# ViTAE-Transformer/SAMRS

Measured on AMD Instinct MI355X. Metric: images/sec (1024^2, vit_h, 32 boxes/img) SAM box->mask, higher is better.
Workload: dtype f16

## Files before the change

samrs_amd/csrc/common.h:

```cpp
#pragma once
#include <hip/hip_runtime.h>
#include <stdint.h>

typedef __attribute__((ext_vector_type(8))) __bf16 bf16x8_t;
typedef __attribute__((ext_vector_type(8))) _Float16 f16x8_t;
typedef __attribute__((ext_vector_type(4))) float f32x4_t;
typedef __attribute__((ext_vector_type(16))) float f32x16_t;

#define SAMRS_WAVE 64

enum { PREC_BF16 = 0, PREC_F16 = 1 };

template <int PREC>
struct ET;

template <>
struct ET<PREC_BF16> {
    static __device__ __forceinline__ uint16_t from_float(float f) {
        __bf16 b = (__bf16)f;
        return __builtin_bit_cast(uint16_t, b);
    }
    static __device__ __forceinline__ float to_float(uint16_t u) {
        return __builtin_bit_cast(float, (uint32_t)u << 16);
    }
// ... 39 lines not shown
}
template <int PREC>
__device__ __forceinline__ uint32_t pack2(float lo, float hi) {
    if (PREC == PREC_F16) {
        lo = __builtin_amdgcn_fmed3f(lo, -65504.0f, 65504.0f);
        hi = __builtin_amdgcn_fmed3f(hi, -65504.0f, 65504.0f);
    }
    return pack2_fast<PREC>(lo, hi);
}

template <int PREC>
__device__ __forceinline__ void split2_pack(float a, float b, uint32_t& hi, uint32_t& lo) {
    hi = pack2<PREC>(a, b);
    const float ha = ET<PREC>::to_float((uint16_t)(hi & 0xffffu)), hb = ET<PREC>::to_float((uint16_t)(hi >> 16));
    lo = pack2<PREC>(a - ha, b - hb);
}

constexpr int MXK = 256;
constexpr int MX_SA_BYTES = 2048, MX_SB_BYTES = 4096;

__device__ __forceinline__ uint32_t fp4_code(float v) {
    const float a = fabsf(v);
    const float step = a >= 4.f ? 2.f : a >= 2.f ? 1.f : 0.5f;
    const float q = fminf(rintf(a / step) * step, 6.f);
    const int idx = (int)(q * 2.f);
    const uint32_t code = idx <= 4 ? (uint32_t)idx : (uint32_t)(idx >> 2) + 4u;
    return code | (v < 0.f ? 8u : 0u);
}
__device__ __forceinline__ int mx_scale_byte(float amax) {
    const int e = (int)((__float_as_uint(amax) >> 23) & 0xffu);
// ... 126 lines not shown
```

samrs_amd/csrc/decoder_kernels.hip:

```cpp
#include "common.h"
#include "kernels.h"
#include "postprocess_value.h"

namespace {

constexpr float TWO_PI = 6.283185307179586f;

__device__ __forceinline__ float pe_channel(const float* __restrict__ gauss, float cx01, float cy01, int ch, int half) {
    const int f = ch < half ? ch : ch - half;
    const float vx = 2.0f * cx01 - 1.0f, vy = 2.0f * cy01 - 1.0f;
    const float a = TWO_PI * (vx * gauss[f] + vy * gauss[half + f]);
    return ch < half ? sinf(a) : cosf(a);
}

__global__ void prompt_tokens_kernel(PromptParams p, float* __restrict__ tokens, float* __restrict__ tokens2, int T, int C) {
    const int j = blockIdx.x, b = blockIdx.y, ch = threadIdx.x;
    const int half = C / 2;
    const bool has_pts = p.point_coords != nullptr;
    const bool has_box = p.boxes != nullptr;
    const int npt = has_pts ? p.n_points + (has_box ? 0 : 1) : 0;
    float v;
    if (j == 0) {
        v = p.iou_token[ch];
    } else if (j < 5) {
// ... 373 lines not shown
        m = mn;
    }
    const float inv = 1.0f / l;
    uint4 o0, o1;
    o0.x = pack2<PREC>(acc[0] * inv, acc[1] * inv);   o0.y = pack2<PREC>(acc[2] * inv, acc[3] * inv);
    o0.z = pack2<PREC>(acc[4] * inv, acc[5] * inv);   o0.w = pack2<PREC>(acc[6] * inv, acc[7] * inv);
    o1.x = pack2<PREC>(acc[8] * inv, acc[9] * inv);   o1.y = pack2<PREC>(acc[10] * inv, acc[11] * inv);
    o1.z = pack2<PREC>(acc[12] * inv, acc[13] * inv); o1.w = pack2<PREC>(acc[14] * inv, acc[15] * inv);
    uint16_t* orow = out + ((size_t)b * tokens + tok) * Ci + h * HD;
    *reinterpret_cast<uint4*>(orow) = o0;
    *reinterpret_cast<uint4*>(orow + 8) = o1;
}

constexpr int I2TF_ROWS = 32;
constexpr int I2TF_AST = 136;

template <int PREC, bool SPLIT>
__global__ __launch_bounds__(256, 2) void i2t_fused_kernel(const uint16_t* __restrict__ qi, int ld, long q_bstride,
                                                        const int* __restrict__ slot_of, const float* __restrict__ kt, const float* __restrict__ vt,
                                                        const uint16_t* __restrict__ w, const uint16_t* __restrict__ w_lo,
                                                        const float* __restrict__ bias,
                                                        const float* __restrict__ resid, long r_bstride,
                                                        const float* __restrict__ gamma, const float* __restrict__ beta, float eps,
                                                        float* __restrict__ outF, uint16_t* __restrict__ outE,
                                                        uint16_t* __restrict__ outE_lo, int T, int tokens, int groups_per_block) {
    constexpr int HD = 16, HEADS = 8, CI = 128, CO = 256, NWV = 4;
    constexpr int KRS = HEADS * I2T_HS;
    extern __shared__ __attribute__((aligned(16))) unsigned char smraw[];
    float* sk = reinterpret_cast<float*>(smraw);
    float* sv = sk + T * KRS;
    float* sp = sv + T * KRS;
    float* ex = sp + 3 * CO;
    uint16_t* At = reinterpret_cast<uint16_t*>(ex + 2 * NWV * I2TF_ROWS);
    uint16_t* Al = At + I2TF_ROWS * I2TF_AST;
    const int tid = threadIdx.x, lane = tid & 63, wave = tid >> 6;
    const int fr = lane & 15, fq = lane >> 4;
    const int b = blockIdx.y;
    for (int i = tid; i < T * CI; i += 256) {
        const int j = i / CI, c = i % CI;
        sk[j * KRS + (c / HD) * I2T_HS + c % HD] = kt[(size_t)b * T * CI + i];
        sv[j * KRS + (c / HD) * I2T_HS + c % HD] = vt[(size_t)b * T * CI + i];
    }
    for (int i = tid; i < CO; i += 256) { sp[i] = bias[i]; sp[CO + i] = gamma[i]; sp[2 * CO + i] = beta[i]; }
    uint4 wf[4][4], wl[SPLIT ? 4 : 1][4];
#pragma unroll
    for (int i = 0; i < 4; ++i)
#pragma unroll
        for (int ks = 0; ks < 4; ++ks) {
            const size_t o = (size_t)(wave * 64 + i * 16 + fr) * CI + ks * 32 + fq * 8;
            wf[i][ks] = *reinterpret_cast<const uint4*>(w + o);
            if constexpr (SPLIT) wl[i][ks] = *reinterpret_cast<const uint4*>(w_lo + o);
        }
    __syncthreads();

    const int tr = tid >> 3, h = tid & 7;
    const int g0 = blockIdx.x * groups_per_block;
    const int ib = slot_of ? slot_of[b] : b;
    const uint16_t* qbase = qi + (size_t)ib * q_bstride * ld + (size_t)tr * ld + h * HD;
    uint4 q0 = make_uint4(0u, 0u, 0u, 0u), q1 = q0;
    if (g0 * I2TF_ROWS < tokens) {
        q0 = *reinterpret_cast<const uint4*>(qbase + (size_t)g0 * I2TF_ROWS * ld);
        q1 = *reinterpret_cast<const uint4*>(qbase + (size_t)g0 * I2TF_ROWS * ld + 8);
    }
    for (int g = g0; g < g0 + groups_per_block; ++g) {
        const int row0 = g * I2TF_ROWS;
        if (row0 >= tokens) break;
        float4 rs[2][4];
#pragma unroll
        for (int mt = 0; mt < 2; ++mt)
#pragma unroll
            for (int i = 0; i < 4; ++i)
                rs[mt][i] = *reinterpret_cast<const float4*>(resid + ((size_t)ib * r_bstride + row0 + mt * 16 + fr) * CO + wave * 64 + i * 16 + 4 * fq);
        {
            const uint32_t qw[8] = {q0.x, q0.y, q0.z, q0.w, q1.x, q1.y, q1.z, q1.w};
            float qf[HD];
#pragma unroll
            for (int c = 0; c < 8; ++c) {
                qf[2 * c] = ET<PREC>::to_float((uint16_t)(qw[c] & 0xffffu)) * 0.25f;
                qf[2 * c + 1] = ET<PREC>::to_float((uint16_t)(qw[c] >> 16)) * 0.25f;
            }
            float m = -INFINITY, l = 0.f, acc[HD];
#pragma unroll
            for (int c = 0; c < HD; ++c) acc[c] = 0.f;
            for (int j = 0; j < T; ++j) {
                float kr[HD], vr[HD];
#pragma unroll
                for (int c4 = 0; c4 < HD / 4; ++c4) {
// ... 11 lines not shown
#pragma unroll
                for (int c = 0; c < HD; ++c) acc[c] = acc[c] * corr + pj * vr[c];
                m = mn;
            }
            const float inv = 1.0f / l;
            uint32_t oh[8], ol[8];
#pragma unroll
            for (int c = 0; c < 8; ++c) split2_pack<PREC>(acc[2 * c] * inv, acc[2 * c + 1] * inv, oh[c], ol[c]);
            *reinterpret_cast<uint4*>(At + tr * I2TF_AST + h * HD) = make_uint4(oh[0], oh[1], oh[2], oh[3]);
            *reinterpret_cast<uint4*>(At + tr * I2TF_AST + h * HD + 8) = make_uint4(oh[4], oh[5], oh[6], oh[7]);
            if constexpr (SPLIT) {
                *reinterpret_cast<uint4*>(Al + tr * I2TF_AST + h * HD) = make_uint4(ol[0], ol[1], ol[2], ol[3]);
                *reinterpret_cast<uint4*>(Al + tr * I2TF_AST + h * HD + 8) = make_uint4(ol[4], ol[5], ol[6], ol[7]);
            }
        }
        __syncthreads();
        if (g + 1 < g0 + groups_per_block && (g + 1) * I2TF_ROWS < tokens) {
            q0 = *reinterpret_cast<const uint4*>(qbase + (size_t)(g + 1) * I2TF_ROWS * ld);
            q1 = *reinterpret_cast<const uint4*>(qbase + (size_t)(g + 1) * I2TF_ROWS * ld + 8);
        }
        float v[2][4][4];
        float s1[2];
#pragma unroll
        for (int mt = 0; mt < 2; ++mt) {
            uint4 af[4], al[SPLIT ? 4 : 1];
#pragma unroll
            for (int ks = 0; ks < 4; ++ks) {
                af[ks] = *reinterpret_cast<const uint4*>(At + (mt * 16 + fr) * I2TF_AST + ks * 32 + fq * 8);
                if constexpr (SPLIT) al[ks] = *reinterpret_cast<const uint4*>(Al + (mt * 16 + fr) * I2TF_AST + ks * 32 + fq * 8);
            }
            s1[mt] = 0.f;
#pragma unroll
            for (int i = 0; i < 4; ++i) {
                f32x4_t a = {0.f, 0.f, 0.f, 0.f};
                if constexpr (SPLIT) {
                    f32x4_t c = {0.f, 0.f, 0.f, 0.f};
#pragma unroll
                    for (int ks = 0; ks < 4; ++ks) c = ET<PREC>::mfma16(wf[i][ks], al[ks], c);
#pragma unroll
                    for (int ks = 0; ks < 4; ++ks) c = ET<PREC>::mfma16(wl[i][ks], af[ks], c);
                    a = c;
                }
#pragma unroll
                for (int ks = 0; ks < 4; ++ks) a = ET<PREC>::mfma16(wf[i][ks], af[ks], a);
                const float4 bb = *reinterpret_cast<const float4*>(sp + wave * 64 + i * 16 + 4 * fq);
                v[mt][i][0] = (a[0] + bb.x) + rs[mt][i].x; v[mt][i][1] = (a[1] + bb.y) + rs[mt][i].y;
                v[mt][i][2] = (a[2] + bb.z) + rs[mt][i].z; v[mt][i][3] = (a[3] + bb.w) + rs[mt][i].w;
                s1[mt] += (v[mt][i][0] + v[mt][i][1]) + (v[mt][i][2] + v[mt][i][3]);
            }
        }
#pragma unroll
        for (int mt = 0; mt < 2; ++mt) {
            s1[mt] += __shfl_xor(s1[mt], 16, 64);
            s1[mt] += __shfl_xor(s1[mt], 32, 64);
            if (fq == 0) ex[wave * I2TF_ROWS + mt * 16 + fr] = s1[mt];
        }
        __syncthreads();
        float mean[2], s2[2];
#pragma unroll
        for (int mt = 0; mt < 2; ++mt) {
            const int r = mt * 16 + fr;
            mean[mt] = ((ex[r] + ex[I2TF_ROWS + r]) + (ex[2 * I2TF_ROWS + r] + ex[3 * I2TF_ROWS + r])) * (1.0f / CO);
            s2[mt] = 0.f;
#pragma unroll
            for (int i = 0; i < 4; ++i)
#pragma unroll
                for (int r4 = 0; r4 < 4; ++r4) { v[mt][i][r4] -= mean[mt]; s2[mt] += v[mt][i][r4] * v[mt][i][r4]; }
            s2[mt] += __shfl_xor(s2[mt], 16, 64);
            s2[mt] += __shfl_xor(s2[mt], 32, 64);
            if (fq == 0) ex[NWV * I2TF_ROWS + wave * I2TF_ROWS + r] = s2[mt];
        }
        __syncthreads();
#pragma unroll
        for (int mt = 0; mt < 2; ++mt) {
            const int r = mt * 16 + fr;
            const float* e2 = ex + NWV * I2TF_ROWS;
            const float rstd = 1.0f / sqrtf(((e2[r] + e2[I2TF_ROWS + r]) + (e2[2 * I2TF_ROWS + r] + e2[3 * I2TF_ROWS + r])) * (1.0f / CO) + eps);
            const size_t orow = (size_t)b * tokens + row0 + r;
#pragma unroll
            for (int i = 0; i < 4; ++i) {
                const int n = wave * 64 + i * 16 + 4 * fq;
                const float4 gm = *reinterpret_cast<const float4*>(sp + CO + n), bt = *reinterpret_cast<const float4*>(sp + 2 * CO + n);
                const float y0 = v[mt][i][0] * rstd * gm.x + bt.x, y1 = v[mt][i][1] * rstd * gm.y + bt.y;
                const float y2 = v[mt][i][2] * rstd * gm.z + bt.z, y3 = v[mt][i][3] * rstd * gm.w + bt.w;
                if (outF) *reinterpret_cast<float4*>(outF + orow * CO + n) = make_float4(y0, y1, y2, y3);
                uint2 o, lo;
                split2_pack<PREC>(y0, y1, o.x, lo.x);
                split2_pack<PREC>(y2, y3, o.y, lo.y);
                *reinterpret_cast<uint2*>(outE + orow * CO + n) = o;
                if (outE_lo) *reinterpret_cast<uint2*>(outE_lo + orow * CO + n) = lo;
            }
        }
    }
}

template <int PREC>
__global__ __launch_bounds__(256) void group_ln_gelu_kernel(const float* __restrict__ in, const float* __restrict__ gamma,
                                                            const float* __restrict__ beta, float eps,
                                                            uint16_t* __restrict__ out, long rows) {
    const int lane = threadIdx.x & 63;
    const long row = (long)blockIdx.x * 4 + (threadIdx.x >> 6);
    if (row >= rows) return;
    const float4 v = reinterpret_cast<const float4*>(in + row * 256)[lane];
    float s = (v.x + v.y) + (v.z + v.w);
#pragma unroll
    for (int off = 8; off > 0; off >>= 1) s += __shfl_xor(s, off, 64);
    const float mean = s * (1.0f / 64.0f);
    const float a = v.x - mean, b = v.y - mean, c = v.z - mean, d = v.w - mean;
// ... 581 lines not shown
        i2t_attention_kernel<PREC_BF16><<<g, b, sh, s>>>((const uint16_t*)qi, ld, bstride, kt, vt, (uint16_t*)out, T, tokens, Ci);
    else
        i2t_attention_kernel<PREC_F16><<<g, b, sh, s>>>((const uint16_t*)qi, ld, bstride, kt, vt, (uint16_t*)out, T, tokens, Ci);
    return hipGetLastError();
}
hipError_t launch_i2t_fused(int prec, const void* qi, int ld, long q_bstride, const float* kt, const float* vt, const void* w,
                            const void* w_lo, const float* bias, const float* resid, long r_bstride, const float* gamma,
                            const float* beta, float eps, float* outF, void* outE, void* outE_lo, int n, int T, int tokens, int Ci,
                            int C, hipStream_t s, const int* slot_of) {
    if (Ci != 128 || C != 256 || T < 1 || T > TOK_MAX || tokens % I2TF_ROWS) return hipErrorInvalidValue;
    const int groups = tokens / I2TF_ROWS;
    int gpb = 4;
    while (gpb > 1 && groups % gpb) gpb >>= 1;
    dim3 g(groups / gpb, n), b(256);
    const bool split = w_lo != nullptr;
    const size_t sh = (size_t)(2 * T * 8 * I2T_HS + 3 * 256 + 2 * 4 * I2TF_ROWS) * sizeof(float) +
                      (size_t)(split ? 2 : 1) * I2TF_ROWS * I2TF_AST * 2;
#define I2TF_LAUNCH(P, S)                                                                                                       \
    i2t_fused_kernel<P, S><<<g, b, sh, s>>>((const uint16_t*)qi, ld, q_bstride, slot_of, kt, vt, (const uint16_t*)w, (const uint16_t*)w_lo, \
                                           bias, resid, r_bstride, gamma, beta, eps, outF, (uint16_t*)outE, (uint16_t*)outE_lo, T, \
                                           tokens, gpb)
    if (prec == PREC_BF16) { if (split) I2TF_LAUNCH(PREC_BF16, true); else I2TF_LAUNCH(PREC_BF16, false); }
    else { if (split) I2TF_LAUNCH(PREC_F16, true); else I2TF_LAUNCH(PREC_F16, false); }
#undef I2TF_LAUNCH
    return hipGetLastError();
}
hipError_t launch_group_ln_gelu(int prec, const float* in, const float* gamma, const float* beta, float eps,
                                void* out, long rows, int groups, int gsize, hipStream_t s) {
    if (groups != 4 || gsize != 64) return hipErrorInvalidValue;
    const int blocks = (int)((rows + 3) / 4);
    if (prec == PREC_BF16) group_ln_gelu_kernel<PREC_BF16><<<blocks, 256, 0, s>>>(in, gamma, beta, eps, (uint16_t*)out, rows);
    else group_ln_gelu_kernel<PREC_F16><<<blocks, 256, 0, s>>>(in, gamma, beta, eps, (uint16_t*)out, rows);
    return hipGetLastError();
}
hipError_t launch_mask_product(int prec, const void* up2, const float* hyper, float* low, int n, int grid,
                               int n_mask_tokens, int sel0, int n_sel, hipStream_t s) {
    if (n_sel > 4 || n_sel < 1) return hipErrorInvalidValue;
    const int S = 4 * grid;
// ... 79 lines not shown
```

samrs_amd/csrc/encoder_kernels.hip:

```cpp
#include "common.h"
#include "kernels.h"

namespace {

__constant__ float c_mean[3] = {123.675f, 116.28f, 103.53f};
__constant__ float c_std[3] = {58.395f, 57.12f, 57.375f};

template <int PREC>
__global__ void patch_im2col_kernel(const uint8_t* __restrict__ img, uint16_t* __restrict__ A, uint16_t* __restrict__ A_lo,
                                    int n_images, int in_h, int in_w, int grid, int patch) {
    const int P2 = patch * patch;
    const int halves = patch / 8;
    const long total = (long)n_images * grid * grid * patch * halves;
    const long t = (long)blockIdx.x * blockDim.x + threadIdx.x;
    if (t >= total) return;
    const int half = t % halves;
    long u = t / halves;
    const int ky = u % patch; u /= patch;
    const int px = u % grid; u /= grid;
    const int py = u % grid;
    const int im = u / grid;
    const int y = py * patch + ky, x0 = px * patch + half * 8;
    float v[3][8];
#pragma unroll
// ... 437 lines not shown
        ah = fmaxf(ah, xhalf_partner(ah));
        al = fmaxf(al, xhalf_partner(al));
        const int bh = mx_scale_byte(ah), bl = mx_scale_byte(al);
        const uint2 ch = make_uint2(fp4_pack8(h, bh), fp4_pack8(h + 8, bh)), cl = make_uint2(fp4_pack8(l, bl), fp4_pack8(l + 8, bl));
        *reinterpret_cast<uint2*>(qh + dt * 16 + 8 * hh) = ch;
        *reinterpret_cast<uint2*>(ql + dt * 16 + 8 * hh) = cl;
        if (hh == 0) {
            const size_t si = mx_scale_index(false, (int)row, head * DT + dt, nst4);
            mx.s_hi[si] = (unsigned char)bh;
            mx.s_lo[si] = (unsigned char)bl;
        }
    }
}

template <int HD>
struct WinCfg {
    static constexpr int WS = 14, N = WS * WS, TK = 2 * WS, NT = N / TK, NP = NT * 32;
    static constexpr int DT = (HD + 31) / 32;
    static constexpr bool ONES = SAMRS_WIN_ONES && DT * 32 > HD;
    __device__ static constexpr int lds_key(int key) { return key + (32 - TK) * (key / TK); }
    static constexpr int VSTR = 228;
    static constexpr int NW = 8, THREADS = NW * 64;
    static constexpr int SSTR = 33;
    static constexpr int K_BYTES = NP * HD * 2;
    static constexpr int VT_BYTES = DT * 32 * VSTR * 2;
    static constexpr int S_BYTES = NW * 32 * SSTR * 4;
    static constexpr int TAB_BYTES = 2 * 32 * HD * 2;
    static constexpr int MAX_D = 1280;
    static constexpr int BIAS_BYTES = 2 * MAX_D * 2;
    static constexpr int LDS_BYTES = K_BYTES + VT_BYTES + S_BYTES + TAB_BYTES + BIAS_BYTES;
};

template <int PREC, int HD, int LO = 0 , int PIPE = 0>
__global__ __launch_bounds__(512) void window_attention_kernel(
    const uint16_t* __restrict__ qkv, const float* __restrict__ qkv_bias, const float* __restrict__ rel_h,
    const float* __restrict__ rel_w, uint16_t* __restrict__ out, int grid, int heads, int n_items,
    uint16_t* __restrict__ out_lo = nullptr , MxOut mx = MxOut(),
    uint32_t lo_heads = 0xffffffffu ,
    int dense = 1 ) {
    using C = WinCfg<HD>;
    constexpr int KS = HD / 16;
    constexpr bool PL = (PIPE & 1) != 0;
    extern __shared__ __attribute__((aligned(16))) unsigned char smem[];
    uint16_t* Ks = reinterpret_cast<uint16_t*>(smem);
    uint16_t* Vt = reinterpret_cast<uint16_t*>(smem + C::K_BYTES);
    float* Scr = reinterpret_cast<float*>(smem + C::K_BYTES + C::VT_BYTES);
    uint16_t* Tab = reinterpret_cast<uint16_t*>(smem + C::K_BYTES + C::VT_BYTES + C::S_BYTES);
    uint16_t* Bia = Tab + 2 * 32 * HD;
// ... 113 lines not shown
        } else WIN_LOAD_V((g_) - 1 - NGK < PV ? (g_) - 1 - NGK : 0);                                                 \
    } while (0)
#define WIN_ISSUE(it_)                                                                                               \
    do {                                                                                                             \
        WIN_HEAD(it_);                                                                                               \
        _Pragma("unroll") for (int g_ = 0; g_ < NGRP; ++g_) WIN_GROUP(g_);                                           \
        if constexpr (PL) WIN_LOAD_Q();                                                                              \
    } while (0)

    __syncthreads();
    if constexpr ((PIPE & 2) != 0) {
        if (__builtin_amdgcn_readfirstlane(threadIdx.x) >= 256) __builtin_amdgcn_s_setprio(1);
    }
    int it = blockIdx.x;
#ifdef WIN_TIMING
    unsigned long long wph[6] = {0, 0, 0, 0, 0, 0}, wprev = __builtin_amdgcn_s_memtime();
    const unsigned long long wstart = wprev;
    int n_done = 0;
#define WIN_STAMP(i_) { const unsigned long long tn_ = __builtin_amdgcn_s_memtime(); wph[i_] += tn_ - wprev; wprev = tn_; }
#else
#define WIN_STAMP(i_)
#endif
    if (it < n_items) WIN_ISSUE(it);
    for (; it < n_items; it += gridDim.x) {
        __syncthreads();
        WIN_STAMP(0)
        if (__any(n_pad != 0u)) {
#pragma unroll
            for (int i = 0; i < PK; ++i) {
                const uint4 kb = *reinterpret_cast<const uint4*>(Bia + n_head * HD + ((tid + i * C::THREADS) % CH) * 8);
                kreg[i] = sel4((n_pad >> i) & 1u, kb, kreg[i]);
// ... 31 lines not shown
        const int qc = min(q, n_nq - 1), qh = slot_row(qc, n_vw), qw = qc - qh * n_vw;
        WIN_STAMP(1)
        __syncthreads();
        WIN_STAMP(2)
        const bool has_next = it + (int)gridDim.x < n_items;
        if (has_next) {
            if (wave_u >= n_strips) WIN_ISSUE(it + (int)gridDim.x);
            else WIN_HEAD(it + (int)gridDim.x);
        }
        WIN_STAMP(3)
#ifdef WIN_TIMING
        ++n_done;
#endif
        if (wave_u >= n_strips) continue;

        float* scr = Scr + wave * 32 * C::SSTR + ql * C::SSTR;
        float RH[PL ? 1 : C::WS], BW[16];
        float* rhs = scr;
        {
            const f32x16_t th = tile_times_qT<PREC, HD>(Tab, lane, qf);
            if constexpr (PL) {
                const f32x16_t tw = tile_times_qT<PREC, HD>(Tab + 32 * HD, lane, qf);
#pragma unroll
                for (int r = 0; r < 16; ++r) scr[acc_row(r, hh)] = tw[r];
                wave_lds_sync();
#pragma unroll
                for (int r = 0; r < 16; ++r) {
                    const int c = acc_row(r, hh);
                    BW[r] = c < C::TK ? scr[qw - c % C::WS + C::WS - 1] * LOG2E_F : -INFINITY;
                }
                wave_lds_sync();
// ... 87 lines not shown
            for (int u = 0; u < 2; ++u) {
                const uint4 pb = pack_p<PREC>(S, u);
#pragma unroll
                for (int dt = 0; dt < C::DT; ++dt) {
                    const uint4 va = load_vt_frag(Vt + (dt * 32 + ql) * C::VSTR + 32 * t, u, hh);
                    O[dt] = ET<PREC>::mfma32(va, pb, O[dt]);
                }
            }
        }
        if constexpr (C::ONES) l_run = ones_row_sum<HD, C::DT>(O, hh);
        else l_run += xhalf_partner(l_run);

#ifdef WIN_TIMING
        asm volatile("" :: "v"(O[0][0]), "v"(O[C::DT - 1][15]), "v"(l_run), "v"(qin), "v"(im), "v"(head));
        WIN_STAMP(5)
        continue;
#endif
        if (qin) {
            const float inv = 1.0f / l_run;
            const size_t orow_i = (size_t)im * img_rows + (size_t)(qoff / (3 * D));
            const size_t obase = orow_i * D + head * HD;
            uint16_t* orow = out + obase;
            if constexpr (LO == 2) store_attention_row_mx<PREC, HD, C::DT>(O, inv, orow, hh, mx, orow_i, head, heads);
            else
#pragma unroll
            for (int dt = 0; dt < C::DT; ++dt)
#pragma unroll
                for (int g = 0; g < 4; ++g) {
                    const int d0 = 32 * dt + 8 * g + 4 * hh;
                    if (d0 < HD) {
                        uint2 o;
                        o.x = pack2_fast<PREC>(O[dt][4 * g + 0] * inv, O[dt][4 * g + 1] * inv);
                        o.y = pack2_fast<PREC>(O[dt][4 * g + 2] * inv, O[dt][4 * g + 3] * inv);
                        *reinterpret_cast<uint2*>(orow + d0) = o;
                        if constexpr (LO == 1) {
                            if ((lo_heads >> (head & 31)) & 1u) {
                                uint2 h, l;
                                split2_pack<PREC>(O[dt][4 * g + 0] * inv, O[dt][4 * g + 1] * inv, h.x, l.x);
                                split2_pack<PREC>(O[dt][4 * g + 2] * inv, O[dt][4 * g + 3] * inv, h.y, l.y);
                                *reinterpret_cast<uint2*>(out_lo + obase + d0) = l;
                            }
                        }
                    }
                }
        }
    }
#ifdef WIN_TIMING
    if (lane == 0) {
        unsigned long long* tp = reinterpret_cast<unsigned long long*>(out) + ((size_t)blockIdx.x * 8 + wave) * 8;
        for (int i = 0; i < 6; ++i) tp[i] = wph[i];
        tp[6] = __builtin_amdgcn_s_memtime() - wstart;
        tp[7] = n_done;
    }
#endif
#undef WIN_ISSUE
#undef WIN_GROUP
#undef WIN_LOAD_V
#undef WIN_LOAD_K
#undef WIN_LOAD_Q
#undef WIN_HEAD
#undef WIN_TOK2
}

__device__ __forceinline__ void glds16_sbase(uint32_t voff, const void* sbase, uint32_t m0v) {
    uint32_t keep;
    asm volatile(
        "s_mov_b32 %0, m0\n\t"
        "s_mov_b32 m0, %3\n\t"
        "s_nop 0\n\t"
        "global_load_lds_dwordx4 %1, %2\n\t"
        "s_mov_b32 m0, %0"
        : "=&s"(keep)
        : "v"(voff), "s"(sbase), "s"(m0v)
        : "memory");
}

template <int HD>
__global__ __launch_bounds__(256) void vt_pack_kernel(const uint16_t* __restrict__ qkv, uint16_t* __restrict__ vt, int heads,
                                                      int ntok) {
    __shared__ uint16_t tile[64][HD + 2];
    const int tiles = ntok / 64;
    const int t = blockIdx.x % tiles, P = blockIdx.x / tiles;
    const int head = P % heads, im = P / heads;
    const int D = heads * HD;
    const uint16_t* src = qkv + ((size_t)im * ntok + (size_t)t * 64) * (3 * D) + 2 * D + head * HD;
    constexpr int CH = HD / 8;
    for (int c = threadIdx.x; c < 64 * CH; c += 256) {
        const int r = c / CH, ch = c % CH;
        const uint4 v = *reinterpret_cast<const uint4*>(src + (size_t)r * (3 * D) + ch * 8);
// ... 19 lines not shown
    static constexpr int DT = (HD + 31) / 32;
    static constexpr int VSTR = KT + 8;
    static constexpr int KSTR = HD + 8;
    static constexpr int K_BYTES = KT * KSTR * 2;
    static constexpr int VT_BYTES = DT * 32 * VSTR * 2;
    static constexpr int NKB = 2, NVB = SAMRS_GLB_SKEW ? 3 : 2;
    static constexpr int KV_BYTES = NKB * K_BYTES + NVB * VT_BYTES;
    static constexpr int SSTR = 33;
    static constexpr int SCR_BYTES = NW * 32 * SSTR * 4;
    static constexpr int UNION_BYTES = KV_BYTES > SCR_BYTES ? KV_BYTES : SCR_BYTES;
    static constexpr int RH_STR = 65;
    static constexpr int RH_BYTES = NW * 32 * RH_STR * 4;
    static constexpr int LDS_BYTES = UNION_BYTES + RH_BYTES;
};

template <int PREC, int HD, int NW, int LO = 0 , int PIPE = 0>
__global__ __launch_bounds__(64 * NW, 2) void global_attention_kernel(
    const uint16_t* __restrict__ qkv, const uint16_t* __restrict__ vt, const float* __restrict__ rel_h,
    const float* __restrict__ rel_w, uint16_t* __restrict__ out, int heads,
    uint16_t* __restrict__ out_lo = nullptr , MxOut mx = MxOut()) {
    using C = GlbCfg<HD, NW>;
    constexpr int KS = HD / 16;
    constexpr int QPB = 32 * NW, NTH = 64 * NW;
    constexpr int G = C::G, NTOK = G * G;
    extern __shared__ __attribute__((aligned(16))) unsigned char smem[];
    float* Scr = reinterpret_cast<float*>(smem);
    auto Kb = [&](int b) { return reinterpret_cast<uint16_t*>(smem + b * C::K_BYTES); };
    auto Vb = [&](int b) { return reinterpret_cast<uint16_t*>(smem + C::NKB * C::K_BYTES + b * C::VT_BYTES); };
    float* RH = reinterpret_cast<float*>(smem + C::UNION_BYTES);

    const int tid = threadIdx.x, lane = tid & 63, wave = tid >> 6;
// ... 234 lines not shown
        if (!SAMRS_GLB_SKEW) {
            asm volatile("s_waitcnt vmcnt(0)" ::: "memory");
            GLB_STAMP(4)
            __syncthreads();
        } else if (grp == 0) {
            asm volatile("s_waitcnt vmcnt(0)" ::: "memory");
            GLB_STAMP(4)
            __builtin_amdgcn_s_barrier();
            asm volatile("" ::: "memory");
        }
        GLB_STAMP(5)
        vb = vb1;
    }

#ifdef GLB_TIMING
    if (lane == 0) {
        unsigned long long* tp = reinterpret_cast<unsigned long long*>(out) + ((size_t)blockIdx.x * 8 + wave) * 8;
        for (int i = 0; i < 6; ++i) tp[i] = tph[i];
        tp[6] = __builtin_amdgcn_s_memtime() - tstart;
        tp[7] = tstart - t_entry;
    }
    asm volatile("" :: "v"(O[0][0]), "v"(O[C::DT - 1][15]), "v"(l_run));
    return;
#endif
    if constexpr (ONES) l_run = ones_row_sum<HD, C::DT>(O, hh);
    else l_run += xhalf_partner(l_run);
    const float inv = 1.0f / l_run;
    const size_t obase = ((size_t)im * NTOK + q) * D + head * HD;
    uint16_t* orow = out + obase;
    if constexpr (LO == 2) store_attention_row_mx<PREC, HD, C::DT>(O, inv, orow, hh, mx, (size_t)im * NTOK + q, head, heads);
    else
#pragma unroll
    for (int dt = 0; dt < C::DT; ++dt)
#pragma unroll
        for (int g = 0; g < 4; ++g) {
            const int d0 = 32 * dt + 8 * g + 4 * hh;
            if (d0 < HD) {
                uint2 o;
                o.x = pack2_fast<PREC>(O[dt][4 * g + 0] * inv, O[dt][4 * g + 1] * inv);
                o.y = pack2_fast<PREC>(O[dt][4 * g + 2] * inv, O[dt][4 * g + 3] * inv);
                *reinterpret_cast<uint2*>(orow + d0) = o;
                if constexpr (LO == 1) {
                    uint2 h, l;
                    split2_pack<PREC>(O[dt][4 * g + 0] * inv, O[dt][4 * g + 1] * inv, h.x, l.x);
                    split2_pack<PREC>(O[dt][4 * g + 2] * inv, O[dt][4 * g + 3] * inv, h.y, l.y);
                    *reinterpret_cast<uint2*>(out_lo + obase + d0) = l;
                }
            }
        }
}

__global__ void neck_im2col_kernel(const uint16_t* __restrict__ in, uint16_t* __restrict__ A, int n_images,
                                   int grid, int C) {
    const int cpr = 9 * C / 8;
    const long total = (long)n_images * grid * grid * cpr;
    const long t = (long)blockIdx.x * blockDim.x + threadIdx.x;
    if (t >= total) return;
    const int ch = t % cpr;
    const long row = t / cpr;
    const int tap = (ch * 8) / C, c0 = (ch * 8) % C;
    const int x = row % grid, y = (row / grid) % grid;
    const long im = row / ((long)grid * grid);
    const int yy = y + tap / 3 - 1, xx = x + tap % 3 - 1;
    uint4 v = make_uint4(0u, 0u, 0u, 0u);
// ... 209 lines not shown
    if (ld_out < D || ld_out % 4 || (ld_out != D && out_lo)) return hipErrorInvalidValue;
    if (n_oc < 0 || n_oc > 32 || (n_oc && (!oc_idx || !out_et || window_mode || ld_out < D + 64))) return hipErrorInvalidValue;
    MxOut mx;
    if (mx_q_hi) {
        if (!mx_q_lo || !mx_s_hi || !mx_s_lo || !out_et || window_mode || D % MXK) return hipErrorInvalidValue;
        mx.q_hi = (unsigned char*)mx_q_hi; mx.q_lo = (unsigned char*)mx_q_lo; mx.s_hi = (unsigned char*)mx_s_hi; mx.s_lo = (unsigned char*)mx_s_lo;
    }
    const int blocks = (rows_out + 3) / 4;
    if (prec == PREC_BF16)
        layernorm_kernel<PREC_BF16><<<blocks, 256, 0, s>>>(X, gamma, beta, eps, (uint16_t*)out_et, out_f32, rows_out, D, window_mode, grid, window, (uint16_t*)out_lo, mx, ld_out, oc_idx, n_oc);
    else
        layernorm_kernel<PREC_F16><<<blocks, 256, 0, s>>>(X, gamma, beta, eps, (uint16_t*)out_et, out_f32, rows_out, D, window_mode, grid, window, (uint16_t*)out_lo, mx, ld_out, oc_idx, n_oc);
    return hipGetLastError();
}

template <int PREC, int HD, int LO = 0>
static hipError_t launch_win(const void* qkv, const float* qb, const float* rh, const float* rw, void* out, int n_images,
                             int grid, int heads, hipStream_t s, void* out_lo = nullptr, MxOut mx = MxOut(), uint32_t lo_heads = 0xffffffffu) {
    using C = WinCfg<HD>;
#ifdef SAMRS_EXPERIMENTS
    static const int pipe = [] { const char* v = getenv("SAMRS_WIN_PIPE"); return v ? atoi(v) & 3 : 0; }();
    auto k = pipe == 3 ? window_attention_kernel<PREC, HD, LO, 3> : pipe == 2 ? window_attention_kernel<PREC, HD, LO, 2>
           : pipe == 1 ? window_attention_kernel<PREC, HD, LO, 1> : window_attention_kernel<PREC, HD, LO, 0>;
#else
    auto k = window_attention_kernel<PREC, HD, LO, 0>;
#endif
    static const int dense = [] { const char* v = getenv("SAMRS_WIN_DENSE"); return (v && atoi(v) == 0) ? 0 : 1; }();
    HIP_CHECK_RET(set_lds(k, C::LDS_BYTES));
    if (heads * HD > C::MAX_D) return hipErrorInvalidValue;
    const int nw = (grid + C::WS - 1) / C::WS;
    const int n_items = n_images * nw * nw * heads;
    static const int n_cu = [] {
        int dev = 0, n = 256;
        if (hipGetDevice(&dev) == hipSuccess) (void)hipDeviceGetAttribute(&n, hipDeviceAttributeMultiprocessorCount, dev);
        return n > 0 ? n : 256;
    }();
    dim3 g(n_items < n_cu ? n_items : n_cu), b(C::THREADS);
    k<<<g, b, C::LDS_BYTES, s>>>((const uint16_t*)qkv, qb, rh, rw, (uint16_t*)out, grid, heads, n_items, (uint16_t*)out_lo, mx, lo_heads,
                                 dense);
    return hipGetLastError();
}
// ... 24 lines not shown
}

static int g_glb_waves = [] { const char* v = getenv("SAMRS_GLB_WAVES"); return (v && atoi(v) == 4) ? 4 : 8; }();

template <int PREC, int HD, int NW, int LO = 0>
static hipError_t launch_glb_nw(const void* qkv, const float* rh, const float* rw, void* out, int n_images,
                                int heads, void* vt_ws, hipStream_t s, void* out_lo = nullptr, MxOut mx = MxOut()) {
    using C = GlbCfg<HD, NW>;
    constexpr int NTOK = C::G * C::G;
#ifdef SAMRS_EXPERIMENTS
    static const bool pipe = [] { const char* v = getenv("SAMRS_GLB_PIPE"); return v ? atoi(v) != 0 : false; }();
    auto k = pipe ? global_attention_kernel<PREC, HD, NW, LO, 1> : global_attention_kernel<PREC, HD, NW, LO, 0>;
#else
    auto k = global_attention_kernel<PREC, HD, NW, LO, 0>;
#endif
    HIP_CHECK_RET(set_lds(k, C::LDS_BYTES));
    dim3 g((NTOK / (32 * NW)) * heads * n_images), b(64 * NW);
    k<<<g, b, C::LDS_BYTES, s>>>((const uint16_t*)qkv, (const uint16_t*)vt_ws, rh, rw, (uint16_t*)out, heads, (uint16_t*)out_lo, mx);
    return hipGetLastError();
}

template <int PREC, int HD>
static hipError_t launch_glb(const void* qkv, const float* rh, const float* rw, void* out, int n_images,
                             int heads, void* vt_ws, hipStream_t s, void* out_lo, MxOut mx) {
    constexpr int NTOK = GlbCfg<HD>::G * GlbCfg<HD>::G;
    vt_pack_kernel<HD><<<n_images * heads * (NTOK / 64), 256, 0, s>>>((const uint16_t*)qkv, (uint16_t*)vt_ws, heads, NTOK);
    HIP_CHECK_RET(hipGetLastError());
    if (mx.q_hi) return launch_glb_nw<PREC, HD, 8, 2>(qkv, rh, rw, out, n_images, heads, vt_ws, s, nullptr, mx);
    if (out_lo) return launch_glb_nw<PREC, HD, 8, 1>(qkv, rh, rw, out, n_images, heads, vt_ws, s, out_lo);
    if (g_glb_waves == 4) return launch_glb_nw<PREC, HD, 4>(qkv, rh, rw, out, n_images, heads, vt_ws, s);
// ... 56 lines not shown
```

Baseline: 149.0.

## Stage attention and i2t outputs through LDS for coalesced row stores

Window and global attention kernels now write their per-wave output tiles into an LDS patch, then emit full 16-byte row chunks so global stores are coalesced. The i2t fused kernel loads residual rows with global_load_lds and stages its LayerNorm output in LDS, so both the fp32 and packed stores become contiguous row writes. All three paths are on by default behind an env switch and alignment checks. The cost is extra LDS traffic, extra barriers and more LDS per block in i2t, which can lower occupancy. Timing instrumentation is also reworked.

```diff
diff --git a/samrs_amd/csrc/common.h b/samrs_amd/csrc/common.h
--- a/samrs_amd/csrc/common.h
+++ b/samrs_amd/csrc/common.h
@@ -77,6 +77,19 @@
     hi = pack2<PREC>(a, b);
     const float ha = ET<PREC>::to_float((uint16_t)(hi & 0xffffu)), hb = ET<PREC>::to_float((uint16_t)(hi >> 16));
     lo = pack2<PREC>(a - ha, b - hb);
+}
+
+__device__ __forceinline__ void glds16_sbase(uint32_t voff, const void* sbase, uint32_t m0v) {
+    uint32_t keep;
+    asm volatile(
+        "s_mov_b32 %0, m0\n\t"
+        "s_mov_b32 m0, %3\n\t"
+        "s_nop 0\n\t"
+        "global_load_lds_dwordx4 %1, %2\n\t"
+        "s_mov_b32 m0, %0"
+        : "=&s"(keep)
+        : "v"(voff), "s"(sbase), "s"(m0v)
+        : "memory");
 }
 
 constexpr int MXK = 256;
diff --git a/samrs_amd/csrc/decoder_kernels.hip b/samrs_amd/csrc/decoder_kernels.hip
--- a/samrs_amd/csrc/decoder_kernels.hip
+++ b/samrs_amd/csrc/decoder_kernels.hip
@@ -411,8 +411,9 @@
 
 constexpr int I2TF_ROWS = 32;
 constexpr int I2TF_AST = 136;
-
-template <int PREC, bool SPLIT>
+constexpr int I2TF_TS = 260;
+
+template <int PREC, bool SPLIT, bool ROWS = false>
 __global__ __launch_bounds__(256, 2) void i2t_fused_kernel(const uint16_t* __restrict__ qi, int ld, long q_bstride,
                                                         const int* __restrict__ slot_of, const float* __restrict__ kt, const float* __restrict__ vt,
                                                         const uint16_t* __restrict__ w, const uint16_t* __restrict__ w_lo,
@@ -424,7 +425,8 @@
     constexpr int HD = 16, HEADS = 8, CI = 128, CO = 256, NWV = 4;
     constexpr int KRS = HEADS * I2T_HS;
     extern __shared__ __attribute__((aligned(16))) unsigned char smraw[];
-    float* sk = reinterpret_cast<float*>(smraw);
+    float* Tl = reinterpret_cast<float*>(smraw);
+    float* sk = Tl + (ROWS ? I2TF_ROWS * I2TF_TS : 0);
     float* sv = sk + T * KRS;
     float* sp = sv + T * KRS;
     float* ex = sp + 3 * CO;
@@ -433,6 +435,13 @@
     const int tid = threadIdx.x, lane = tid & 63, wave = tid >> 6;
     const int fr = lane & 15, fq = lane >> 4;
     const int b = blockIdx.y;
+#ifdef I2T_TIMING
+    unsigned long long iph[5] = {0, 0, 0, 0, 0}, iprev = __builtin_amdgcn_s_memtime();
+    int i_groups = 0;
+#define I2T_STAMP(i_) { const unsigned long long tn_ = __builtin_amdgcn_s_memtime(); iph[i_] += tn_ - iprev; iprev = tn_; }
+#else
+#define I2T_STAMP(i_)
+#endif
     for (int i = tid; i < T * CI; i += 256) {
         const int j = i / CI, c = i % CI;
         sk[j * KRS + (c / HD) * I2T_HS + c % HD] = kt[(size_t)b * T * CI + i];
@@ -459,15 +468,27 @@
         q0 = *reinterpret_cast<const uint4*>(qbase + (size_t)g0 * I2TF_ROWS * ld);
         q1 = *reinterpret_cast<const uint4*>(qbase + (size_t)g0 * I2TF_ROWS * ld + 8);
     }
+    const float* rbase = resid + ((size_t)ib * r_bstride + __builtin_amdgcn_readfirstlane(wave) * 8) * CO;
+    const uint32_t tl_row0 = (uint32_t)(uintptr_t)(__attribute__((address_space(3))) void*)Tl +
+                             (uint32_t)__builtin_amdgcn_readfirstlane(wave) * 8u * (I2TF_TS * 4);
+#ifdef I2T_TIMING
+    iprev = __builtin_amdgcn_s_memtime();
+#endif
     for (int g = g0; g < g0 + groups_per_block; ++g) {
         const int row0 = g * I2TF_ROWS;
         if (row0 >= tokens) break;
         float4 rs[2][4];
+        if constexpr (ROWS) {
+#pragma unroll
+            for (int k = 0; k < 8; ++k) glds16_sbase(16u * lane, rbase + ((size_t)row0 + k) * CO, tl_row0 + k * (I2TF_TS * 4));
+        } else {
 #pragma unroll
         for (int mt = 0; mt < 2; ++mt)
 #pragma unroll
             for (int i = 0; i < 4; ++i)
                 rs[mt][i] = *reinterpret_cast<const float4*>(resid + ((size_t)ib * r_bstride + row0 + mt * 16 + fr) * CO + wave * 64 + i * 16 + 4 * fq);
+        }
+        I2T_STAMP(0)
         {
             const uint32_t qw[8] = {q0.x, q0.y, q0.z, q0.w, q1.x, q1.y, q1.z, q1.w};
             float qf[HD];
@@ -509,8 +530,11 @@
                 *reinterpret_cast<uint4*>(Al + tr * I2TF_AST + h * HD + 8) = make_uint4(ol[4], ol[5], ol[6], ol[7]);
             }
         }
+        if constexpr (ROWS) asm volatile("s_waitcnt vmcnt(0)" ::: "memory");
+        I2T_STAMP(1)
         __syncthreads();
-        if (g + 1 < g0 + groups_per_block && (g + 1) * I2TF_ROWS < tokens) {
+        const bool has_next = g + 1 < g0 + groups_per_block && (g + 1) * I2TF_ROWS < tokens;
+        if (has_next) {
             q0 = *reinterpret_cast<const uint4*>(qbase + (size_t)(g + 1) * I2TF_ROWS * ld);
             q1 = *reinterpret_cast<const uint4*>(qbase + (size_t)(g + 1) * I2TF_ROWS * ld + 8);
         }
@@ -539,11 +563,16 @@
 #pragma unroll
                 for (int ks = 0; ks < 4; ++ks) a = ET<PREC>::mfma16(wf[i][ks], af[ks], a);
                 const float4 bb = *reinterpret_cast<const float4*>(sp + wave * 64 + i * 16 + 4 * fq);
+                if constexpr (ROWS) rs[mt][i] = *reinterpret_cast<const float4*>(Tl + (mt * 16 + fr) * I2TF_TS + wave * 64 + i * 16 + 4 * fq);
                 v[mt][i][0] = (a[0] + bb.x) + rs[mt][i].x; v[mt][i][1] = (a[1] + bb.y) + rs[mt][i].y;
                 v[mt][i][2] = (a[2] + bb.z) + rs[mt][i].z; v[mt][i][3] = (a[3] + bb.w) + rs[mt][i].w;
                 s1[mt] += (v[mt][i][0] + v[mt][i][1]) + (v[mt][i][2] + v[mt][i][3]);
             }
         }
+#ifdef I2T_TIMING
+        asm volatile("" :: "v"(v[0][0][0]), "v"(v[1][3][3]), "v"(s1[0]), "v"(s1[1]));
+#endif
+        I2T_STAMP(2)
 #pragma unroll
         for (int mt = 0; mt < 2; ++mt) {
             s1[mt] += __shfl_xor(s1[mt], 16, 64);
@@ -566,6 +595,7 @@
             if (fq == 0) ex[NWV * I2TF_ROWS + wave * I2TF_ROWS + r] = s2[mt];
         }
         __syncthreads();
+        I2T_STAMP(3)
 #pragma unroll
         for (int mt = 0; mt < 2; ++mt) {
             const int r = mt * 16 + fr;
@@ -578,15 +608,56 @@
                 const float4 gm = *reinterpret_cast<const float4*>(sp + CO + n), bt = *reinterpret_cast<const float4*>(sp + 2 * CO + n);
                 const float y0 = v[mt][i][0] * rstd * gm.x + bt.x, y1 = v[mt][i][1] * rstd * gm.y + bt.y;
                 const float y2 = v[mt][i][2] * rstd * gm.z + bt.z, y3 = v[mt][i][3] * rstd * gm.w + bt.w;
+                if constexpr (ROWS) {
+                    *reinterpret_cast<float4*>(Tl + r * I2TF_TS + n) = make_float4(y0, y1, y2, y3);
+                } else {
                 if (outF) *reinterpret_cast<float4*>(outF + orow * CO + n) = make_float4(y0, y1, y2, y3);
                 uint2 o, lo;
                 split2_pack<PREC>(y0, y1, o.x, lo.x);
                 split2_pack<PREC>(y2, y3, o.y, lo.y);
                 *reinterpret_cast<uint2*>(outE + orow * CO + n) = o;
                 if (outE_lo) *reinterpret_cast<uint2*>(outE_lo + orow * CO + n) = lo;
-            }
-        }
-    }
+                }
+            }
+        }
+        if constexpr (ROWS) {
+            __syncthreads();
+            int ln = lane;
+            asm volatile("" : "+v"(ln));
+            const size_t orow0 = (size_t)b * tokens + row0 + wave * 8;
+            if (outF) {
+#pragma unroll
+                for (int k = 0; k < 8; ++k)
+                    *reinterpret_cast<float4*>(outF + (orow0 + k) * CO + 4 * ln) = *reinterpret_cast<const float4*>(Tl + (wave * 8 + k) * I2TF_TS + 4 * ln);
+            }
+#pragma unroll
+            for (int k = 0; k < 4; ++k) {
+                const int r = 2 * k + (ln >> 5), c = 8 * (ln & 31);
+                const float4 ya = *reinterpret_cast<const float4*>(Tl + (wave * 8 + r) * I2TF_TS + c);
+                const float4 yb = *reinterpret_cast<const float4*>(Tl + (wave * 8 + r) * I2TF_TS + c + 4);
+                uint4 o, lo;
+                split2_pack<PREC>(ya.x, ya.y, o.x, lo.x);
+                split2_pack<PREC>(ya.z, ya.w, o.y, lo.y);
+                split2_pack<PREC>(yb.x, yb.y, o.z, lo.z);
+                split2_pack<PREC>(yb.z, yb.w, o.w, lo.w);
+                *reinterpret_cast<uint4*>(outE + (orow0 + r) * CO + c) = o;
+                if (outE_lo) *reinterpret_cast<uint4*>(outE_lo + (orow0 + r) * CO + c) = lo;
+            }
+        }
+        I2T_STAMP(4)
+#ifdef I2T_TIMING
+        ++i_groups;
+#endif
+    }
+#ifdef I2T_TIMING
+    if (lane == 0) {
+        unsigned long long* tp = reinterpret_cast<unsigned long long*>(outE + (size_t)gridDim.y * tokens * CO) +
+                                 (((size_t)blockIdx.y * gridDim.x + blockIdx.x) * NWV + wave) * 8;
+        for (int i = 0; i < 5; ++i) tp[i] = iph[i];
+        tp[5] = i_groups;
+    }
+#endif
+#undef I2T_STAMP
 }
 
 template <int PREC>
@@ -1198,14 +1269,23 @@
     while (gpb > 1 && groups % gpb) gpb >>= 1;
     dim3 g(groups / gpb, n), b(256);
     const bool split = w_lo != nullptr;
+    constexpr bool I2T_ROW_STORES_DEFAULT = true;
+    static const bool row_stores = [] { const char* v = getenv("SAMRS_ROW_STORES"); return v ? atoi(v) != 0 : I2T_ROW_STORES_DEFAULT; }();
+    const bool rows = row_stores && ((uintptr_t)resid % 16) == 0 && ((uintptr_t)outF % 16) == 0 && ((uintptr_t)outE % 16) == 0 &&
+                      ((uintptr_t)outE_lo % 16) == 0;
     const size_t sh = (size_t)(2 * T * 8 * I2T_HS + 3 * 256 + 2 * 4 * I2TF_ROWS) * sizeof(float) +
-                      (size_t)(split ? 2 : 1) * I2TF_ROWS * I2TF_AST * 2;
-#define I2TF_LAUNCH(P, S)                                                                                                       \
-    i2t_fused_kernel<P, S><<<g, b, sh, s>>>((const uint16_t*)qi, ld, q_bstride, slot_of, kt, vt, (const uint16_t*)w, (const uint16_t*)w_lo, \
+                      (size_t)(split ? 2 : 1) * I2TF_ROWS * I2TF_AST * 2 + (rows ? (size_t)I2TF_ROWS * I2TF_TS * sizeof(float) : 0);
+#define I2TF_LAUNCH(P, S, R)                                                                                                    \
+    do {                                                                                                                        \
+        if (sh > 64 * 1024) HIP_CHECK_RET(hipFuncSetAttribute((const void*)i2t_fused_kernel<P, S, R>, hipFuncAttributeMaxDynamicSharedMemorySize, (int)sh)); \
+        i2t_fused_kernel<P, S, R><<<g, b, sh, s>>>((const uint16_t*)qi, ld, q_bstride, slot_of, kt, vt, (const uint16_t*)w, (const uint16_t*)w_lo, \
                                            bias, resid, r_bstride, gamma, beta, eps, outF, (uint16_t*)outE, (uint16_t*)outE_lo, T, \
-                                           tokens, gpb)
-    if (prec == PREC_BF16) { if (split) I2TF_LAUNCH(PREC_BF16, true); else I2TF_LAUNCH(PREC_BF16, false); }
-    else { if (split) I2TF_LAUNCH(PREC_F16, true); else I2TF_LAUNCH(PREC_F16, false); }
+                                           tokens, gpb);                                                                        \
+    } while (0)
+#define I2TF_LAUNCH_R(P, S) do { if (rows) I2TF_LAUNCH(P, S, true); else I2TF_LAUNCH(P, S, false); } while (0)
+    if (prec == PREC_BF16) { if (split) I2TF_LAUNCH_R(PREC_BF16, true); else I2TF_LAUNCH_R(PREC_BF16, false); }
+    else { if (split) I2TF_LAUNCH_R(PREC_F16, true); else I2TF_LAUNCH_R(PREC_F16, false); }
+#undef I2TF_LAUNCH_R
 #undef I2TF_LAUNCH
     return hipGetLastError();
 }
diff --git a/samrs_amd/csrc/encoder_kernels.hip b/samrs_amd/csrc/encoder_kernels.hip
--- a/samrs_amd/csrc/encoder_kernels.hip
+++ b/samrs_amd/csrc/encoder_kernels.hip
@@ -475,6 +475,48 @@
 }
 
 template <int HD>
+struct RowPatch {
+    static constexpr int CH = HD / 8;
+    static constexpr int RSTR = HD * 2 + 16;
+    static constexpr int BYTES = 32 * RSTR;
+    static constexpr int NI = (32 * CH + 63) / 64;
+    static_assert(HD % 8 == 0, "a row segment is a whole number of 16-byte chunks");
+};
+
+template <int PREC, int HD, int DT>
+__device__ __forceinline__ void store_attention_rows(const f32x16_t (&O)[DT], float inv, unsigned char* patch, int row, int lane,
+                                                     uint16_t* __restrict__ out, int head, int D) {
+    using R = RowPatch<HD>;
+    const int hh = lane >> 5, ql = lane & 31;
+    if (hh == 0) *reinterpret_cast<int*>(patch + ql * R::RSTR + HD * 2) = row;
+#pragma unroll
+    for (int dt = 0; dt < DT; ++dt)
+#pragma unroll
+        for (int g = 0; g < 4; ++g) {
+            const int d0 = 32 * dt + 8 * g + 4 * hh;
+            if (d0 < HD) {
+                uint2 o;
+                o.x = pack2_fast<PREC>(O[dt][4 * g + 0] * inv, O[dt][4 * g + 1] * inv);
+                o.y = pack2_fast<PREC>(O[dt][4 * g + 2] * inv, O[dt][4 * g + 3] * inv);
+                *reinterpret_cast<uint2*>(patch + ql * R::RSTR + d0 * 2) = o;
+            }
+        }
+    wave_lds_sync();
+    uint16_t* dst = out + head * HD;
+#pragma unroll
+    for (int i = 0; i < R::NI; ++i) {
+        const int c = lane + 64 * i;
+        if (32 * R::CH % 64 == 0 || c < 32 * R::CH) {
+            const int r = c / R::CH, ch = c % R::CH;
+            const int prow = *reinterpret_cast<const int*>(patch + r * R::RSTR + HD * 2);
+            const uint4 v = *reinterpret_cast<const uint4*>(patch + r * R::RSTR + ch * 16);
+            if (prow >= 0) *reinterpret_cast<uint4*>(dst + (size_t)prow * D + ch * 8) = v;
+        }
+    }
+    wave_lds_sync();
+}
+
+template <int HD>
 struct WinCfg {
     static constexpr int WS = 14, N = WS * WS, TK = 2 * WS, NT = N / TK, NP = NT * 32;
     static constexpr int DT = (HD + 31) / 32;
@@ -485,14 +527,16 @@
     static constexpr int SSTR = 33;
     static constexpr int K_BYTES = NP * HD * 2;
     static constexpr int VT_BYTES = DT * 32 * VSTR * 2;
-    static constexpr int S_BYTES = NW * 32 * SSTR * 4;
+    static constexpr int SCR_W = 32 * SSTR * 4 > RowPatch<HD>::BYTES ? 32 * SSTR * 4 : RowPatch<HD>::BYTES;
+    static constexpr int S_BYTES = NW * SCR_W;
     static constexpr int TAB_BYTES = 2 * 32 * HD * 2;
     static constexpr int MAX_D = 1280;
     static constexpr int BIAS_BYTES = 2 * MAX_D * 2;
     static constexpr int LDS_BYTES = K_BYTES + VT_BYTES + S_BYTES + TAB_BYTES + BIAS_BYTES;
 };
 
-template <int PREC, int HD, int LO = 0 , int PIPE = 0>
+template <int PREC, int HD, int LO = 0 , int PIPE = 0,
+          int ROWS = 0 >
 __global__ __launch_bounds__(512) void window_attention_kernel(
     const uint16_t* __restrict__ qkv, const float* __restrict__ qkv_bias, const float* __restrict__ rel_h,
     const float* __restrict__ rel_w, uint16_t* __restrict__ out, int grid, int heads, int n_items,
@@ -636,7 +680,7 @@
     }
     int it = blockIdx.x;
 #ifdef WIN_TIMING
-    unsigned long long wph[6] = {0, 0, 0, 0, 0, 0}, wprev = __builtin_amdgcn_s_memtime();
+    unsigned long long wph[7] = {0, 0, 0, 0, 0, 0, 0}, wprev = __builtin_amdgcn_s_memtime();
     const unsigned long long wstart = wprev;
     int n_done = 0;
 #define WIN_STAMP(i_) { const unsigned long long tn_ = __builtin_amdgcn_s_memtime(); wph[i_] += tn_ - wprev; wprev = tn_; }
@@ -698,7 +742,7 @@
 #endif
         if (wave_u >= n_strips) continue;
 
-        float* scr = Scr + wave * 32 * C::SSTR + ql * C::SSTR;
+        float* scr = Scr + wave * (C::SCR_W / 4) + ql * C::SSTR;
         float RH[PL ? 1 : C::WS], BW[16];
         float* rhs = scr;
         {
@@ -816,8 +860,12 @@
 #ifdef WIN_TIMING
         asm volatile("" :: "v"(O[0][0]), "v"(O[C::DT - 1][15]), "v"(l_run), "v"(qin), "v"(im), "v"(head));
         WIN_STAMP(5)
-        continue;
-#endif
+#endif
+        if constexpr (ROWS != 0 && LO == 0) {
+            const int orow_i = qin ? (int)((size_t)im * img_rows) + qoff / (3 * D) : -1;
+            store_attention_rows<PREC, HD, C::DT>(O, 1.0f / l_run, reinterpret_cast<unsigned char*>(Scr) + wave * C::SCR_W, orow_i, lane,
+                                                  out, head, D);
+        } else
         if (qin) {
             const float inv = 1.0f / l_run;
             const size_t orow_i = (size_t)im * img_rows + (size_t)(qoff / (3 * D));
@@ -846,13 +894,15 @@
                     }
                 }
         }
+        WIN_STAMP(6)
     }
 #ifdef WIN_TIMING
     if (lane == 0) {
-        unsigned long long* tp = reinterpret_cast<unsigned long long*>(out) + ((size_t)blockIdx.x * 8 + wave) * 8;
-        for (int i = 0; i < 6; ++i) tp[i] = wph[i];
-        tp[6] = __builtin_amdgcn_s_memtime() - wstart;
-        tp[7] = n_done;
+        const size_t out_rows = (size_t)(n_items / (nw * nw * heads)) * img_rows;
+        unsigned long long* tp = reinterpret_cast<unsigned long long*>(out + out_rows * D) + ((size_t)blockIdx.x * 8 + wave) * 16;
+        for (int i = 0; i < 7; ++i) tp[i] = wph[i];
+        tp[7] = __builtin_amdgcn_s_memtime() - wstart;
+        tp[8] = n_done;
     }
 #endif
 #undef WIN_ISSUE
@@ -862,19 +912,6 @@
 #undef WIN_LOAD_Q
 #undef WIN_HEAD
 #undef WIN_TOK2
-}
-
-__device__ __forceinline__ void glds16_sbase(uint32_t voff, const void* sbase, uint32_t m0v) {
-    uint32_t keep;
-    asm volatile(
-        "s_mov_b32 %0, m0\n\t"
-        "s_mov_b32 m0, %3\n\t"
-        "s_nop 0\n\t"
-        "global_load_lds_dwordx4 %1, %2\n\t"
-        "s_mov_b32 m0, %0"
-        : "=&s"(keep)
-        : "v"(voff), "s"(sbase), "s"(m0v)
-        : "memory");
 }
 
 template <int HD>
@@ -924,7 +961,7 @@
     static constexpr int LDS_BYTES = UNION_BYTES + RH_BYTES;
 };
 
-template <int PREC, int HD, int NW, int LO = 0 , int PIPE = 0>
+template <int PREC, int HD, int NW, int LO = 0 , int PIPE = 0, int ROWS = 0 >
 __global__ __launch_bounds__(64 * NW, 2) void global_attention_kernel(
     const uint16_t* __restrict__ qkv, const uint16_t* __restrict__ vt, const float* __restrict__ rel_h,
     const float* __restrict__ rel_w, uint16_t* __restrict__ out, int heads,
@@ -1189,14 +1226,9 @@
     }
 
 #ifdef GLB_TIMING
-    if (lane == 0) {
-        unsigned long long* tp = reinterpret_cast<unsigned long long*>(out) + ((size_t)blockIdx.x * 8 + wave) * 8;
-        for (int i = 0; i < 6; ++i) tp[i] = tph[i];
-        tp[6] = __builtin_amdgcn_s_memtime() - tstart;
-        tp[7] = tstart - t_entry;
-    }
+    const unsigned long long t_loop = __builtin_amdgcn_s_memtime() - tstart;
     asm volatile("" :: "v"(O[0][0]), "v"(O[C::DT - 1][15]), "v"(l_run));
-    return;
+    const unsigned long long t_w0 = __builtin_amdgcn_s_memtime();
 #endif
     if constexpr (ONES) l_run = ones_row_sum<HD, C::DT>(O, hh);
     else l_run += xhalf_partner(l_run);
@@ -1204,7 +1236,11 @@
     const size_t obase = ((size_t)im * NTOK + q) * D + head * HD;
     uint16_t* orow = out + obase;
     if constexpr (LO == 2) store_attention_row_mx<PREC, HD, C::DT>(O, inv, orow, hh, mx, (size_t)im * NTOK + q, head, heads);
-    else
+    else if constexpr (ROWS != 0 && LO == 0) {
+        static_assert(32 * C::RH_STR * 4 >= RowPatch<HD>::BYTES && (C::UNION_BYTES % 16) == 0 && (32 * C::RH_STR * 4) % 16 == 0, "row patch");
+        store_attention_rows<PREC, HD, C::DT>(O, inv, reinterpret_cast<unsigned char*>(RH) + wave * (32 * C::RH_STR * 4), im * NTOK + q, lane,
+                                              out, head, D);
+    } else
 #pragma unroll
     for (int dt = 0; dt < C::DT; ++dt)
 #pragma unroll
@@ -1223,6 +1259,17 @@
                 }
             }
         }
+#ifdef GLB_TIMING
+    const unsigned long long t_write = __builtin_amdgcn_s_memtime() - t_w0;
+    if (lane == 0) {
+        const size_t out_rows = (size_t)(gridDim.x / QB / heads) * NTOK;
+        unsigned long long* tp = reinterpret_cast<unsigned long long*>(out + out_rows * D) + ((size_t)blockIdx.x * NW + wave) * 16;
+        for (int i = 0; i < 6; ++i) tp[i] = tph[i];
+        tp[6] = t_loop;
+        tp[7] = tstart - t_entry;
+        tp[8] = t_write;
+    }
+#endif
 }
 
 __global__ void neck_im2col_kernel(const uint16_t* __restrict__ in, uint16_t* __restrict__ A, int n_images,
@@ -1462,6 +1509,14 @@
     return hipGetLastError();
 }
 
+constexpr bool WIN_ROW_STORES_DEFAULT = true;
+constexpr bool GLB_ROW_STORES_DEFAULT = true;
+static bool attention_row_stores(bool dflt, const void* out, int head_dim, int heads, size_t rows) {
+    static const int env = [] { const char* v = getenv("SAMRS_ROW_STORES"); return v ? (atoi(v) != 0 ? 1 : 0) : -1; }();
+    const bool on = env < 0 ? dflt : env != 0;
+    return on && ((uintptr_t)out % 16) == 0 && (head_dim * 2) % 16 == 0 && (heads * head_dim * 2) % 16 == 0 && rows < (size_t)1 << 31;
+}
+
 template <int PREC, int HD, int LO = 0>
 static hipError_t launch_win(const void* qkv, const float* qb, const float* rh, const float* rw, void* out, int n_images,
                              int grid, int heads, hipStream_t s, void* out_lo = nullptr, MxOut mx = MxOut(), uint32_t lo_heads = 0xffffffffu) {
@@ -1473,6 +1528,16 @@
 #else
     auto k = window_attention_kernel<PREC, HD, LO, 0>;
 #endif
+    if constexpr (LO == 0) {
+        if (attention_row_stores(WIN_ROW_STORES_DEFAULT, out, HD, heads, (size_t)n_images * grid * grid)) {
+#ifdef SAMRS_EXPERIMENTS
+            k = pipe == 3 ? window_attention_kernel<PREC, HD, LO, 3, 1> : pipe == 2 ? window_attention_kernel<PREC, HD, LO, 2, 1>
+              : pipe == 1 ? window_attention_kernel<PREC, HD, LO, 1, 1> : window_attention_kernel<PREC, HD, LO, 0, 1>;
+#else
+            k = window_attention_kernel<PREC, HD, LO, 0, 1>;
+#endif
+        }
+    }
     static const int dense = [] { const char* v = getenv("SAMRS_WIN_DENSE"); return (v && atoi(v) == 0) ? 0 : 1; }();
     HIP_CHECK_RET(set_lds(k, C::LDS_BYTES));
     if (heads * HD > C::MAX_D) return hipErrorInvalidValue;
@@ -1527,6 +1592,15 @@
 #else
     auto k = global_attention_kernel<PREC, HD, NW, LO, 0>;
 #endif
+    if constexpr (LO == 0) {
+        if (attention_row_stores(GLB_ROW_STORES_DEFAULT, out, HD, heads, (size_t)n_images * NTOK)) {
+#ifdef SAMRS_EXPERIMENTS
+            k = pipe ? global_attention_kernel<PREC, HD, NW, LO, 1, 1> : global_attention_kernel<PREC, HD, NW, LO, 0, 1>;
+#else
+            k = global_attention_kernel<PREC, HD, NW, LO, 0, 1>;
+#endif
+        }
+    }
     HIP_CHECK_RET(set_lds(k, C::LDS_BYTES));
     dim3 g((NTOK / (32 * NW)) * heads * n_images), b(64 * NW);
     k<<<g, b, C::LDS_BYTES, s>>>((const uint16_t*)qkv, (const uint16_t*)vt_ws, rh, rw, (uint16_t*)out, heads, (uint16_t*)out_lo, mx);
```

Result: no change. 150.0 (median of 2 runs) (+0.7%).
